# stone-d-chen/ffvvc

Measured on AMD Instinct MI355X. Metric: decoded frames/sec (4K/8K 10-bit VVC) per GPU, higher is better.
Workload: dtype u16

## Files before the change

### ffvvc_amd/csrc/intra.hip

```cpp
#include <type_traits>
#include "common.hpp"
#include "pk16.hpp"
#include "wave.hpp"
#include "runtime.hpp"
#include "resid_math.hpp"
#include "../../include/vvc_mi355.h"

namespace vvc355 {

#define VVC355_TABLE(type, name, count) __device__ static const type i_tab_##name[count] __attribute__((aligned(16)))
#include "tables.inc"
#undef VVC355_TABLE

#ifdef VVC355_RECON_PROF
__device__ unsigned long long vvc355_recon_prof[64];
__device__ __forceinline__ unsigned long long *rprof_lds() { __shared__ unsigned long long p[64]; return p; }
#define RPROF_NOW() wall_clock64()
#define RPROF_ADD(slot, t0) do { unsigned long long *p_ = rprof_lds(); p_[slot] = p_[slot] + (unsigned long long)(wall_clock64() - (t0)); } while (0)
#define RPROF_INC(slot) do { unsigned long long *p_ = rprof_lds(); p_[slot] = p_[slot] + 1ull; } while (0)
__device__ unsigned long long vvc355_recon_trace[4096 * 8];
#define RTRACE(rs, slot, v) do { vvc355_recon_trace[((rs) & 4095) * 8 + (slot)] = (unsigned long long)(v); } while (0)
#else
#define RTRACE(rs, slot, v) do { } while (0)
#define RPROF_NOW() 0ull
// ... 126 lines not shown
    int base;
    __device__ __forceinline__ int ld(int off) const { return p[base + off]; }
    __device__ __forceinline__ void st(int off, int v) const { p[base + off] = (uint16_t)v; }
    __device__ __forceinline__ LPix at(int off) const { return LPix{ p, base + off }; }
    __device__ __forceinline__ void st4(int off, int a, int b, int c, int d) const
    {
        uint32_t *q = (uint32_t *)(p + base + off);
        q[0] = (uint32_t)a | ((uint32_t)b << 16);
        q[1] = (uint32_t)c | ((uint32_t)d << 16);
    }
    __device__ __forceinline__ void ld4(int off, int *v) const
    {
        const uint32_t *q = (const uint32_t *)(p + base + off);
        const uint32_t a = q[0], b = q[1];
        v[0] = (int)(a & 0xffff); v[1] = (int)(a >> 16); v[2] = (int)(b & 0xffff); v[3] = (int)(b >> 16);
    }
};

template <int BD> __device__ __forceinline__ GPix<BD> pick3(int c, GPix<BD> a, GPix<BD> b, GPix<BD> d) { return GPix<BD>{ c == 0 ? a.p : c == 1 ? b.p : d.p }; }
__device__ __forceinline__ LPix pick3(int c, LPix a, LPix b, LPix d) { return LPix{ a.p, c == 0 ? a.base : c == 1 ? b.base : d.base }; }
__device__ __forceinline__ StripRef pick3(int c, StripRef a, StripRef b, StripRef d)
{
    return StripRef{ a.p + (c == 0 ? 0 : c == 1 ? (int)(b.p - a.p) : (int)(d.p - a.p)), c == 0 ? a.pitch : c == 1 ? b.pitch : d.pitch, c == 0 ? a.x0s : c == 1 ? b.x0s : d.x0s, false };
}

struct IntraTabsLds {
    uint32_t angle_inv[32];
    uint32_t luma_filter[64];
    uint8_t mip4[1024], mip8[1024], mip16[2688];
};
struct GTabs {
    __device__ __forceinline__ uint32_t angle_inv(int aidx) const { return intra_angle_entry(aidx); }
    __device__ __forceinline__ uint32_t filt4(int e) const { uint32_t d; __builtin_memcpy(&d, i_tab_intra_luma_filter + e * 4, 4); return d; }
    __device__ __forceinline__ const uint8_t *mip(int size_id) const
    {
        return size_id == 0 ? i_tab_mip_matrix_4x4 : size_id == 1 ? i_tab_mip_matrix_8x8 : i_tab_mip_matrix_16x16;
    }
};
struct LTabs {
    const IntraTabsLds *t;
    __device__ __forceinline__ uint32_t angle_inv(int aidx) const { return (uint32_t)__builtin_amdgcn_readfirstlane((int)t->angle_inv[aidx]); }
    __device__ __forceinline__ uint32_t filt4(int e) const { return t->luma_filter[e]; }
    __device__ __forceinline__ const uint8_t *mip(int size_id) const { return size_id == 0 ? t->mip4 : size_id == 1 ? t->mip8 : t->mip16; }
};
struct LTabsLane {
    const IntraTabsLds *t;
// ... 1243 lines not shown
}


namespace vvc355 {

struct ReconLds {
    uint16_t arr[3][4][kEdgeLen];
    int scratch[3][16];
    int prm[2][8];
    uint32_t rmap[2][2][2][32];
    uint32_t cmdbuf[2][64 * 10];
    int luma_done;
    int bc[8];
    IntraTabsLds tabs;
};
struct ReconCtx { int ctb_up, ctb_left, ctb_up_left, end_of_tiles_x, ox, oy; };

__device__ __forceinline__ int recon_run(uint32_t line, int from)
{
    const uint32_t m = (uint32_t)__builtin_amdgcn_readfirstlane((int)line) >> from;
    return m == ~0u ? 32 : __builtin_ctz(~m);
}
typedef uint32_t ReconMaps[2][2][32];
__device__ int recon_top_available(const vvc355_recon_frame &f, const ReconCtx &cx, const ReconMaps &rmap, int cu_x0, int x, int y, int target, int c_idx)
{
    const int hs = c_idx ? f.hs : 0, vs = c_idx ? f.vs : 0;
    const int end_of_ctb_x = ((cu_x0 >> f.ctb_log2) + 1) << f.ctb_log2;
    const int y0b = y & ((1 << (f.ctb_log2 - vs)) - 1);
    const int max_x = min(f.width, end_of_ctb_x) >> hs;
    if (!y0b) {
        if (!cx.ctb_up)
            return 0;
        target = min(target, (cx.end_of_tiles_x >> hs) - x);
        if (f.wpp)
            target = min(target, (end_of_ctb_x >> hs) - x);
        return target;
    }
    target = max(0, min(target, max_x - x));
    const int ux = ((x << hs) - cx.ox) >> 2, uy = (((y - 1) << vs) - cx.oy) >> 2;
    const int end = (cx.ox + ((ux + recon_run(rmap[c_idx > 0][0][uy], ux)) << 2)) >> hs;
    return max(0, min(target, end - x));
}
__device__ int recon_left_available(const vvc355_recon_frame &f, const ReconCtx &cx, const ReconMaps &rmap, int cu_y0, int x, int y, int target, int c_idx)
{
    const int hs = c_idx ? f.hs : 0, vs = c_idx ? f.vs : 0;
    const int x0b = x & ((1 << (f.ctb_log2 - hs)) - 1);
    const int end_of_ctb_y = ((cu_y0 >> f.ctb_log2) + 1) << f.ctb_log2;
    const int max_y = min(f.height, end_of_ctb_y) >> vs;
    if (!x0b && !cx.ctb_left)
        return 0;
    target = max(0, min(target, max_y - y));
    if (!x0b)
        return target;
    const int ux = (((x - 1) << hs) - cx.ox) >> 2, uy = ((y << vs) - cx.oy) >> 2;
    const int end = (cx.oy + ((uy + recon_run(rmap[c_idx > 0][1][ux], uy)) << 2)) >> vs;
    return max(0, min(target, end - y));
}
__host__ __device__ inline int wide_angle_mode(int isp_split, int c_idx, int tb_w, int tb_h, int cb_w, int cb_h, int mode)
{
    const int nw = (!isp_split || c_idx) ? tb_w : cb_w, nh = (!isp_split || c_idx) ? tb_h : cb_h;
    const int d = ilog2i(nw) - ilog2i(nh), wh_ratio = d < 0 ? -d : d;
    const int mx = wh_ratio > 1 ? 8 + 2 * wh_ratio : 8, mn = wh_ratio > 1 ? 60 - 2 * wh_ratio : 60;
    if (nw > nh && mode >= 2 && mode < mx)
        return mode + 65;
    if (nh > nw && mode <= 66 && mode > mn)
        return mode - 67;
// ... 189 lines not shown
        group_sync<64>();
    }
    asm volatile("s_waitcnt vmcnt(0)" ::: "memory");
    __syncthreads();
    if (role == 0) {
        __builtin_amdgcn_fence(__ATOMIC_RELEASE, "agent");
        asm volatile("s_waitcnt vmcnt(0)" ::: "memory");
        __hip_atomic_store(&state[kReconFlags + n_ctus + rs], 1, __ATOMIC_RELAXED, __HIP_MEMORY_SCOPE_AGENT);
        __hip_atomic_store(&state[kReconFlags + rs], 1, __ATOMIC_RELAXED, __HIP_MEMORY_SCOPE_AGENT);
        RTRACE(rs, 2, wall_clock64()); RTRACE(rs, 4, wall_clock64()); RTRACE(rs, 5, wall_clock64());
        RTRACE(rs, 6, ctu.flags | ((unsigned long long)ctu.n_cmd << 8)); 
    }
}

template <int BD, bool TILE>
__device__ __forceinline__ bool recon_one_ctu(const vvc355_recon_frame &f, ReconLds &L, uint16_t *tiles, const int role, const int tid)
{
    using px_t = typename Px<BD>::type;
    using PX = typename std::conditional<TILE, LPix, GPix<BD>>::type;
    VVC355_GLOBAL int *state = (VVC355_GLOBAL int *)f.state;
    if (role == 0) {
        const int t = __hip_atomic_fetch_add(&state[0], tid == 0 ? 1 : 0, __ATOMIC_RELAXED, __HIP_MEMORY_SCOPE_AGENT);
        L.bc[0] = __builtin_amdgcn_readfirstlane(t);
        recon_luma_done_set(L, 0);
    }
    __syncthreads();
    const int ticket = __builtin_amdgcn_readfirstlane(L.bc[0]);
    if (ticket >= f.n_work)
        return false;
    const int rs = __builtin_amdgcn_readfirstlane(gld<int>((const int *)f.order + ticket));
    const vvc355_recon_ctu *ctus = (const vvc355_recon_ctu *)f.ctus;
    const vvc355_recon_ctu ctu = load_uniform(ctus + rs);
    const int ncx = f.ctb_width, ry = rs / ncx, rx = rs - ry * ncx;
    const int ctb = 1 << f.ctb_log2;
    ReconCtx cx;
    {
        const int16_t *slice_idx = (const int16_t *)f.slice_idx, *col_bd = (const int16_t *)f.ctb_to_col_bd, *row_bd = (const int16_t *)f.ctb_to_row_bd;
        const bool left_tile = rx > 0 && gld<int16_t>(col_bd + rx) != gld<int16_t>(col_bd + rx - 1);
        const bool upper_tile = ry > 0 && gld<int16_t>(row_bd + ry) != gld<int16_t>(row_bd + ry - 1);
        const bool upper_slice = ry > 0 && gld<int16_t>(slice_idx + rs) != gld<int16_t>(slice_idx + rs - ncx);
        cx.end_of_tiles_x = f.width;
        if (gld<int16_t>(col_bd + rx) != gld<int16_t>(col_bd + rx + 1))
            cx.end_of_tiles_x = min(rx * ctb + ctb, f.width);
        cx.ctb_left = rx > 0 && !left_tile;
        cx.ctb_up = ry > 0 && !upper_tile && !upper_slice;
        cx.ctb_up_left = cx.ctb_left && cx.ctb_up;
        cx.ox = rx * ctb; cx.oy = ry * ctb;
// ... 11 lines not shown
    const int cw0 = min(ctb, f.width - rx * ctb), ch0 = min(ctb, f.height - ry * ctb);
    if constexpr (TILE) {
#pragma unroll
        for (int c = 0; c < 3; c++) {
            const int sh = c ? 1 : 0, pitch = c ? kBodyChromaP : kBodyLumaP, spitch = c ? kStripChromaP : kStripLumaP;
            const int ox = (rx * ctb) >> sh, oy = (ry * ctb) >> sh;
            if ((c == 0) == (role == 0)) {
                if (c == 0)
                    recon_body_load<BD, 5>(tiles + kTileOff[c], pitch, (const uint8_t *)f.plane[c], f.stride[c], ox, oy, cw0, ch0, f.width, f.height, tid);
                else
                    recon_body_load<BD, 4>(tiles + kTileOff[c], pitch, (const uint8_t *)f.plane[c], f.stride[c], ox, oy, cw0 >> 1, ch0 >> 1, f.width >> 1, f.height >> 1, tid);
            }
            const LPix px{ tiles, kTileOff[c] - oy * pitch + (kApr - ox) };
            const StripRef sx{ tiles + kStripOff[c], spitch, ox - kApr, false };
            if (c == 0) { pl0 = px; st0 = sx; } else if (c == 1) { pl1 = px; st1 = sx; } else { pl2 = px; st2 = sx; }
        }
        ps0 = kBodyLumaP; ps1 = kBodyChromaP;
    }
    const vvc355_recon_cmd *cmds = (const vvc355_recon_cmd *)f.cmds + ctu.first_cmd;
    const int ctb_mask = ctb - 1;
    constexpr int CMD_DW = (int)sizeof(vvc355_recon_cmd) / 4;
    static_assert(CMD_DW == 10, "cmdbuf holds windows of 10-dword commands");
    const uint32_t n_cmd = ctu.n_cmd;
    uint16_t (*arr)[kEdgeLen] = L.arr[role];
    const LTabs tabs{ &L.tabs };
    VVC355_LDS uint32_t *cbuf = (VVC355_LDS uint32_t *)L.cmdbuf[role];
    auto load_window = [&](uint32_t base, uint32_t *all_kinds, auto plan) -> unsigned long long {
        const uint32_t n_dw = min(64u, n_cmd - base) * CMD_DW;
        const uint32_t *g = (const uint32_t *)(cmds + base);
        uint32_t v[CMD_DW];
#pragma unroll
        for (int u = 0; u < CMD_DW; u++)
            v[u] = (uint32_t)tid + 64u * u < n_dw ? gld<uint32_t>(g + tid + 64 * u) : 0u;
#pragma unroll
        for (int u = 0; u < CMD_DW; u++)
            cbuf[tid + 64 * u] = v[u];
        group_sync<64>();
        const uint32_t kinds = cbuf[tid * CMD_DW + 6];
        *all_kinds = kinds;
        const unsigned long long m = __ballot(base + (uint32_t)tid < n_cmd && ((((kinds >> 16) & 0xff) > 0) == (role == 1)) && ((kinds >> 8) & 0xff) != VVC355_RECON_MARK);
        if constexpr (decltype(plan)::value) {
            const bool mine = (m >> tid) & 1;
            ReconPlan P;
            if (mine) {
                uint32_t q[CMD_DW], qn[CMD_DW] = {};
#pragma unroll
                for (int i = 0; i < CMD_DW; i++) q[i] = cbuf[tid * CMD_DW + i];
                bool twin = false;
                if (TILE && tid < 63 && ((m >> (tid + 1)) & 1)) {
#pragma unroll
                    for (int i = 2; i < 9; i++) qn[i] = cbuf[(tid + 1) * CMD_DW + i];
                    twin = recon_plan_twin(q, qn);
                }
                const ReconPlanFrame pf = { f.hs, f.vs, f.ctb_log2, { ps0, ps1 }, TILE };
                P = recon_plan(q, twin, pf, cx, LTabsLane{ &L.tabs });
            }
            group_sync<64>();
            if (mine) {
#pragma unroll
                for (int i = 0; i < CMD_DW; i++) cbuf[tid * CMD_DW + i] = P.d[i];
            }
            group_sync<64>();
        }
        return m;
    };
    {
        ReconMaps &rmap = L.rmap[role];
        ((uint32_t *)rmap)[tid] = 0;
        ((uint32_t *)rmap)[tid + 64] = 0;
        uint32_t *cmd_dw = (uint32_t *)cmds;
        for (uint32_t base = 0; base < n_cmd; base += 64) {
            uint32_t kinds;
            (void)load_window(base, &kinds, std::false_type{});
            const uint32_t kind_l = (kinds >> 8) & 0xff, type_l = ((kinds >> 16) & 0xff) > 0;
            const bool in_l = base + (uint32_t)tid < n_cmd;
            const bool mine = type_l == (uint32_t)role;
            const bool scaled_l = in_l && mine && kind_l == VVC355_RECON_RESID && ((cbuf[tid * CMD_DW + 8] >> 8) & 8);
            unsigned long long todo = __ballot(in_l && ((kind_l == VVC355_RECON_MARK && (role == 1 || type_l == 0)) ||
                                                        (mine && (kind_l == VVC355_RECON_PRED || kind_l == VVC355_RECON_CCLM)) || scaled_l));
            while (todo) {
                const int k = __builtin_ctzll(todo);
                todo &= todo - 1;
                const uint32_t q2 = __builtin_amdgcn_readfirstlane(cbuf[k * CMD_DW + 2]), q3 = __builtin_amdgcn_readfirstlane(cbuf[k * CMD_DW + 3]);
                const uint32_t q4 = __builtin_amdgcn_readfirstlane(cbuf[k * CMD_DW + 4]), q6 = __builtin_amdgcn_readfirstlane(cbuf[k * CMD_DW + 6]);
                const int x0 = (int16_t)(q2 & 0xffff), y0 = (int16_t)(q2 >> 16), cw_ = (int16_t)(q3 & 0xffff), ch_ = (int16_t)(q3 >> 16);
                const int cu_x0 = (int16_t)(q4 & 0xffff), cu_y0 = (int16_t)(q4 >> 16);
                const int kind = (q6 >> 8) & 0xff, c_idx = (q6 >> 16) & 0xff;
                if (kind == VVC355_RECON_MARK) {
                    const int ux = (x0 - cx.ox) >> 2, uy = (y0 - cx.oy) >> 2, uw = max(1, cw_ >> 2), uh = max(1, ch_ >> 2);
                    const int i = tid & 31, t = tid >> 5;
                    const int span = t ? uw : uh, first = t ? ux : uy, len = t ? uh : uw, at = t ? uy : ux;
                    if (i < span)
                        rmap[c_idx > 0][t][first + i] |= (len >= 32 ? ~0u : ((1u << len) - 1)) << at;
                    __builtin_amdgcn_fence(__ATOMIC_RELEASE, "wavefront");
                    continue;
                }
// ... 1 lines not shown
                if (kind == VVC355_RECON_PRED) {
                    const int hs = c_idx ? f.hs : 0, vs = c_idx ? f.vs : 0;
                    dw9 = (uint32_t)(uint16_t)__builtin_amdgcn_readfirstlane(recon_left_available(f, cx, rmap, cu_y0, x0 >> hs, y0 >> vs, 16384, c_idx)) |
                          (uint32_t)(uint16_t)__builtin_amdgcn_readfirstlane(recon_top_available(f, cx, rmap, cu_x0, x0 >> hs, y0 >> vs, 16384, c_idx)) << 16;
                } else if (kind == VVC355_RECON_CCLM) {
                    dw9 = (uint32_t)(uint16_t)__builtin_amdgcn_readfirstlane(recon_left_available(f, cx, rmap, cu_y0, x0 >> f.hs, y0 >> f.vs, 16384, 1)) |
                          (uint32_t)(uint16_t)__builtin_amdgcn_readfirstlane(recon_top_available(f, cx, rmap, cu_x0, x0 >> f.hs, y0 >> f.vs, 16384, 1)) << 16;
                    bits = (__builtin_amdgcn_readfirstlane(recon_left_available(f, cx, rmap, cu_y0, x0, y0, 1, 0)) != 0 ? 1u : 0u) |
                           (__builtin_amdgcn_readfirstlane(recon_top_available(f, cx, rmap, cu_x0, x0, y0, 1, 0)) != 0 ? 2u : 0u);
                } else {
                    const int size_y = min(ctb, 64), xv = cu_x0 & ~(size_y - 1), yv = cu_y0 & ~(size_y - 1);
                    bits = (__builtin_amdgcn_readfirstlane(recon_left_available(f, cx, rmap, cu_y0, xv, yv, 1, 0)) != 0 ? 1u : 0u) |
                           (__builtin_amdgcn_readfirstlane(recon_top_available(f, cx, rmap, cu_x0, xv, yv, 1, 0)) != 0 ? 2u : 0u);
                }
                if (tid == 0) {
                    uint32_t *g = cmd_dw + (size_t)(base + k) * CMD_DW;
                    gst<uint32_t>(g + 9, dw9);
                    gst<uint8_t>((uint8_t *)(g + 8) + 2, (uint8_t)bits);
                }
            }
        }
        asm volatile("s_waitcnt vmcnt(0)" ::: "memory");
    }
    const unsigned long long t_wait = RPROF_NOW();
    if (role == 0) { RTRACE(rs, 0, wall_clock64()); RTRACE(rs, 6, ctu.flags | ((unsigned long long)ctu.n_cmd << 8)); }
    {
        const int n_ctus = ncx * f.ctb_height;
        const int dep[4] = { rx > 0 ? rs - 1 : -1, (rx > 0 && ry > 0) ? rs - ncx - 1 : -1, ry > 0 ? rs - ncx : -1, (ry > 0 && rx + 1 < ncx) ? rs - ncx + 1 : -1 };
#pragma unroll
        for (int d = 0; d < 4; d++) {
            if (dep[d] < 0 || __builtin_amdgcn_readfirstlane(gld<uint32_t>(&ctus[dep[d]].n_cmd)) == 0)
                continue;
            if (role == 0 && (__builtin_amdgcn_readfirstlane(gld<uint32_t>(&ctus[dep[d]].flags)) & VVC355_RECON_CTU_LIGHT))
                continue;
            VVC355_GLOBAL int *flag = &state[kReconFlags + (role == 0 ? n_ctus : 0) + dep[d]];
            while (__builtin_amdgcn_readfirstlane(__hip_atomic_load(flag, __ATOMIC_RELAXED, __HIP_MEMORY_SCOPE_AGENT)) == 0)
                __builtin_amdgcn_s_sleep(4);
        }
        __builtin_amdgcn_fence(__ATOMIC_ACQUIRE, "agent");
        asm volatile("s_waitcnt vmcnt(0)" ::: "memory");
    }
    RPROF_ADD(1 + 32 * role, t_wait);
    RPROF_INC(0 + 32 * role);
    RTRACE(rs, role ? 3 : 1, wall_clock64());
    const unsigned long long t_load = RPROF_NOW();
    if constexpr (TILE) {
#pragma unroll
        for (int c = 0; c < 3; c++) {
            const int sh = c ? 1 : 0;
            if ((c == 0) == (role == 0))
                recon_edges_load<BD>(tiles + kTileOff[c], c ? kBodyChromaP : kBodyLumaP, tiles + kStripOff[c], c ? kStripChromaP : kStripLumaP, (const uint8_t *)f.plane[c], f.stride[c],
                                     (rx * ctb) >> sh, (ry * ctb) >> sh, ctb >> sh, ch0 >> sh, f.width >> sh, f.height >> sh, tid);
        }
        asm volatile("s_waitcnt vmcnt(0)" ::: "memory");
        group_sync<64>();
    } else {
        pl0 = GPix<BD>{ (uint8_t *)f.plane[0] }; pl1 = GPix<BD>{ (uint8_t *)f.plane[1] }; pl2 = GPix<BD>{ (uint8_t *)f.plane[2] };
        ps0 = f.stride[0] / (int)sizeof(px_t); ps1 = f.stride[1] / (int)sizeof(px_t);
    }

    RPROF_ADD(2 + 32 * role, t_load);
    const unsigned long long t_loop = RPROF_NOW();
#ifdef VVC355_RECON_PROF
    const long long c_loop = clock64();
#endif
    uint32_t win = (uint32_t)0 - 64u, kinds_unused;
    unsigned long long mask = 0;
    auto advance = [&]() -> int {
        while (!mask) {
            if (win + 64 >= n_cmd)
                return -1;
            win += 64;
            mask = load_window(win, &kinds_unused, std::true_type{});
        }
        const int bit = __builtin_ctzll(mask);
        mask &= mask - 1;
        return (int)win + bit;
    };
    auto load_cmd = [&](int idx) -> uint32_t { return cbuf[(idx - (int)win) * CMD_DW + min(tid, CMD_DW - 1)]; };
    int i0 = -1;
    auto shift = [&]() {
        i0 = advance();
        if (role == 0)
            recon_luma_done_set(L, i0 >= 0 ? i0 : (int)n_cmd);
    };
    int4 pre[4] = {};
    int pre_k = -1;
    int lmcs_xv = -1, lmcs_yv = -1, lmcs_scale = 0;
    int n_shift = 1;
    for (;;) {
        do shift(); while (--n_shift);
        if (i0 < 0)
            break;
        n_shift = 1;
        const uint32_t k = (uint32_t)i0;
        const int i1 = mask ? (int)win + __builtin_ctzll(mask) : -1;
        const uint32_t d0 = load_cmd(i0), d1 = i1 >= 0 ? load_cmd(i1) : 0u;
        uint32_t p[CMD_DW];
#pragma unroll
        for (int i = 0; i < CMD_DW; i++) p[i] = (uint32_t)__builtin_amdgcn_readlane((int)d0, i);
        const int kind = (int)((p[6] >> 8) & 0xff);
        if (i1 >= 0) {
            const uint32_t n6 = (uint32_t)__builtin_amdgcn_readlane((int)d1, 6);
            if (((n6 >> 8) & 0xff) == VVC355_RECON_RESID && pre_k != i0) {
                const uint64_t ptr = (uint32_t)__builtin_amdgcn_readlane((int)d1, 0) | ((uint64_t)(uint32_t)__builtin_amdgcn_readlane((int)d1, 1) << 32);
                const uint32_t wh = (uint32_t)__builtin_amdgcn_readlane((int)d1, 3);
                const int nn = (int)(wh & 0xffff) * (int)(wh >> 16);
#pragma unroll
                for (int u = 0; u < 4; u++)
                    if (tid * 4 + 256 * u < nn)
                        pre[u] = gld<int4>((const int *)ptr + tid * 4 + 256 * u);
                pre_k = i1;
            }
        }
        const unsigned long long t_cmd = RPROF_NOW();
        if (kind == VVC355_RECON_PRED) {
            const IntraSetup su = recon_plan_setup(p);
            const uint32_t fl = p[8] >> 16;
            RPROF_ADD(6 + 32 * role, t_cmd);
            if (TILE && (fl & kPlanTwin)) {
                if constexpr (TILE) {
                    const int half = tid >> 5;
                    const LPix plane2{ pl1.p, half ? pl2.base : pl1.base };
                    StripRef sr2{ st1.p + (half ? (int)(st2.p - st1.p) : 0), st1.pitch, st1.x0s, (fl & kPlanStrip) != 0 };
                    intra_pred_run<BD, 32>(su, plane2, ps1, L.arr[1 + half], L.scratch[1 + half], tid & 31, sr2, tabs);
                    group_sync<64>();
                    n_shift = 2;
                }
            } else {
                const PX plane = pick3(su.c_idx, pl0, pl1, pl2);
                StripRef sr = pick3(su.c_idx, st0, st1, st2);
                sr.on = (fl & kPlanStrip) != 0;
                intra_pred_run<BD, 64>(su, plane, su.c_idx ? ps1 : ps0, arr, L.scratch[role], tid, sr, tabs);
                if (TILE) group_sync<64>(); else recon_sync_mem();
            }
        } else if (kind == VVC355_RECON_CCLM) {
            while (recon_luma_done_get(L) < (int)k)
                __builtin_amdgcn_s_sleep(1);
            group_sync<64>();
            vvc355_cclm_job j = {};
            j.x0 = (int16_t)(p[2] & 0xffff); j.y0 = (int16_t)(p[2] >> 16); j.width = (int16_t)(p[3] & 0xffff); j.height = (int16_t)(p[3] >> 16);
            j.top_avail_c = (int16_t)(p[9] >> 16);
            j.left_avail_c = (int16_t)(p[9] & 0xffff);
            j.mode = (uint8_t)(p[6] & 0xff); j.hs = f.hs; j.vs = f.vs;
            j.avail_l = (uint8_t)(p[7] & 0xff);
            j.avail_t = (uint8_t)((p[7] >> 8) & 0xff);
            j.collocated = f.collocated;
            j.ctu_boundary = (uint8_t)((p[7] >> 16) & 0xff);
            StripRef s0 = st0, s1 = st1, s2 = st2;
            s0.on = s1.on = s2.on = TILE && j.ctu_boundary;
            cclm_body<BD, 64>(j, pl0, ps0, pl1, pl2, ps1, ps1, L.prm[1], tid, s0, s1, s2);
            if (TILE) group_sync<64>(); else recon_sync_mem();
        } else if (kind == VVC355_RECON_CIIP) {
            const int c_idx = (int)((p[4] >> 8) & 0xff), lw = (int)(p[4] & 0xff), w = 1 << lw, n = (int)p[5];
            const int stride = c_idx ? ps1 : ps0, iw = (int)((p[4] >> 16) & 0xff);
            const PX dst = pick3(c_idx, pl0, pl1, pl2).at((int)p[2]);
            const uint8_t *inter = (const uint8_t *)(p[0] | ((uint64_t)p[1] << 32));
            for (int i = tid; i < n; i += 64) {
                const int o = (i >> lw) * stride + (i & (w - 1));
                dst.st(o, (dst.ld(o) * iw + ld_px<BD>(inter, i) * (4 - iw) + 2) >> 2);
            }
            if (TILE) group_sync<64>(); else recon_sync_mem();
        } else {
            const int c_idx = (int)((p[4] >> 8) & 0xff), lw = (int)(p[4] & 0xff), w = 1 << lw, n = (int)p[5];
            const int stride = c_idx ? ps1 : ps0, joint = (int)((p[4] >> 16) & 0xff);
            const PX dst = pick3(c_idx, pl0, pl1, pl2).at((int)p[2]);
            const int *res = (const int *)(p[0] | ((uint64_t)p[1] << 32));
            const bool have = pre_k == (int)k;
            const bool scaled = (p[4] >> 24) != 0;
            const int xv = (int16_t)(p[7] & 0xffff), yv = (int16_t)(p[7] >> 16);
            if (scaled && (lmcs_xv != xv || lmcs_yv != yv)) {
                while (recon_luma_done_get(L) < (int)k)
                    __builtin_amdgcn_s_sleep(1);
                group_sync<64>();
                const int size_y = min(ctb, 64);
                lmcs_xv = xv; lmcs_yv = yv;
                const bool avail_t = (p[8] >> 17) & 1, avail_l = (p[8] >> 16) & 1;
                StripRef s0 = st0;
                s0.on = TILE && (lmcs_yv & ctb_mask) == 0;
                int v = 0;
                if (tid < size_y) {
                    if (avail_l)
                        v += pl0.ld((lmcs_yv + min(tid, min(f.height - lmcs_yv, size_y) - 1)) * ps0 + lmcs_xv - 1);
                    if (avail_t) {
                        const int xx = lmcs_xv + min(tid, min(f.width - lmcs_xv, size_y) - 1);
                        v += s0.on ? s0.at(xx, -1) : pl0.ld((lmcs_yv - 1) * ps0 + xx);
                    }
                }
#pragma unroll
                for (int sft = 32; sft; sft >>= 1)
                    v += __shfl_xor(v, sft, 64);
                const int cnt = (avail_l ? size_y : 0) + (avail_t ? size_y : 0);
                const int avg = cnt ? (v + (cnt >> 1)) >> ilog2i(cnt) : 1 << (BD - 1);
                lmcs_scale = lmcs_scale_of_avg((const vvc355_lmcs_model *)f.lmcs_model, avg, tid);
            }
            auto resid_of = [&](int r) {
                if (joint & 1)
                    r = (r * ((joint & 2) ? -1 : 1)) >> ((joint >> 2) & 1);
                if (scaled) {
                    const int v = clip_intp2(r, BD);
                    r = v > 0 ? (v * lmcs_scale + (1 << 10)) >> 11 : -((-v * lmcs_scale + (1 << 10)) >> 11);
                }
                return r;
            };
            auto add4 = [&](int i, const int4 r4) {
                const int r[4] = { r4.x, r4.y, r4.z, r4.w };
                const int o = (i >> lw) * stride + (i & (w - 1));
                int d[4];
                dst.ld4(o, d);
#pragma unroll
                for (int q = 0; q < 4; q++)
                    d[q] = clip_px<BD>(d[q] + resid_of(r[q]));
                dst.st4(o, d[0], d[1], d[2], d[3]);
            };
            if (w < 4) {
                for (int i = tid; i < n; i += 64) {
                    const int o = (i >> lw) * stride + (i & (w - 1));
                    dst.st(o, clip_px<BD>(dst.ld(o) + resid_of(gld<int>(res + i))));
                }
            } else {
#pragma unroll
                for (int u = 0; u < 4; u++) {
                    const int i = tid * 4 + 256 * u;
                    if (i < n)
                        add4(i, have ? pre[u] : gld<int4>(res + i));
                }
                for (int i = tid * 4 + 1024; i < n; i += 256)
                    add4(i, gld<int4>(res + i));
            }
            if (TILE) group_sync<64>(); else recon_sync_mem();
        }
        RPROF_ADD(9 + kind + 32 * role, t_cmd);
        RPROF_INC(17 + kind + 32 * role);
    }
    RPROF_ADD(3 + 32 * role, t_loop);
#ifdef VVC355_RECON_PROF
    { unsigned long long *p_ = rprof_lds(); p_[7 + 32 * role] = p_[7 + 32 * role] + (unsigned long long)(clock64() - c_loop); }
#endif
    if (role == 0) {
        if constexpr (TILE) {
            const int nk = cw0 >> 2, nr = ch0;
            recon_tile_store<BD, 5>(tiles + kTileOff[0], kBodyLumaP, (uint8_t *)f.plane[0], f.stride[0], rx * ctb, ry * ctb, max(nr - kApr, 0), nr, 0, nk, tid);
            recon_tile_store<BD, 0>(tiles + kTileOff[0], kBodyLumaP, (uint8_t *)f.plane[0], f.stride[0], rx * ctb, ry * ctb, 0, max(nr - kApr, 0), nk - 1, nk, tid);
        }
        asm volatile("s_waitcnt vmcnt(0)" ::: "memory");
        __builtin_amdgcn_fence(__ATOMIC_RELEASE, "agent");
        asm volatile("s_waitcnt vmcnt(0)" ::: "memory");
        __hip_atomic_store(&state[kReconFlags + ncx * f.ctb_height + rs], 1, __ATOMIC_RELAXED, __HIP_MEMORY_SCOPE_AGENT);
        RTRACE(rs, 2, wall_clock64());
    } else {
        RTRACE(rs, 4, wall_clock64());
    }
    const unsigned long long t_join = RPROF_NOW();
    __syncthreads();
    RPROF_ADD(4 + 32 * role, t_join);
    const unsigned long long t_store = RPROF_NOW();
    if constexpr (TILE) {
#pragma unroll
        for (int c = 0; c < 3; c++) {
            const int sh = c ? 1 : 0, pitch = c ? kBodyChromaP : kBodyLumaP, nk = cw0 >> (2 + sh), nr = ch0 >> sh;
            if ((c == 0) != (role == 0))
                continue;
            uint8_t *plane = (uint8_t *)f.plane[c];
            if (c == 0) {
            } else {
                recon_tile_store<BD, 4>(tiles + kTileOff[c], pitch, plane, f.stride[c], (rx * ctb) >> sh, (ry * ctb) >> sh, max(nr - kApr, 0), nr, 0, nk, tid);
                recon_tile_store<BD, 0>(tiles + kTileOff[c], pitch, plane, f.stride[c], (rx * ctb) >> sh, (ry * ctb) >> sh, 0, max(nr - kApr, 0), nk - 1, nk, tid);
            }
        }
    }
    asm volatile("s_waitcnt vmcnt(0)" ::: "memory");
    __syncthreads();
    if (role == 0) {
        __builtin_amdgcn_fence(__ATOMIC_RELEASE, "agent");
        asm volatile("s_waitcnt vmcnt(0)" ::: "memory");
// ... 111 lines not shown
```

Before: 612.8.

## Specialize recon command walk per role at compile time

Wraps the per-CTU wait, edge load, command loop and luma store in a generic lambda instantiated separately for the luma role and the chroma role, so role checks and plane/stride selection (pick_role) become compile-time constants. It also force-inlines the top/left availability helpers and initializes the luma-done marker to -1 instead of 0. The aim is to cut divergent branching, register pressure and scalar overhead in the hot command loop. In exchange it roughly doubles code size and may raise instruction-cache pressure. The -1 init also changes CCLM/LMCS wait semantics for the first command.

After: 630.8 (median of 6 runs). +2.9%, better.

```diff
diff --git a/ffvvc_amd/csrc/intra.hip b/ffvvc_amd/csrc/intra.hip
--- a/ffvvc_amd/csrc/intra.hip
+++ b/ffvvc_amd/csrc/intra.hip
@@ -172,6 +172,14 @@
 __device__ __forceinline__ StripRef pick3(int c, StripRef a, StripRef b, StripRef d)
 {
     return StripRef{ a.p + (c == 0 ? 0 : c == 1 ? (int)(b.p - a.p) : (int)(d.p - a.p)), c == 0 ? a.pitch : c == 1 ? b.pitch : d.pitch, c == 0 ? a.x0s : c == 1 ? b.x0s : d.x0s, false };
+}
+template <int ROLE, int BD> __device__ __forceinline__ GPix<BD> pick_role(int c, GPix<BD> a, GPix<BD> b, GPix<BD> d) { return GPix<BD>{ ROLE == 0 ? a.p : c == 1 ? b.p : d.p }; }
+template <int ROLE> __device__ __forceinline__ LPix pick_role(int c, LPix a, LPix b, LPix d) { return LPix{ a.p, ROLE == 0 ? a.base : c == 1 ? b.base : d.base }; }
+template <int ROLE> __device__ __forceinline__ StripRef pick_role(int c, StripRef a, StripRef b, StripRef d)
+{
+    if (ROLE == 0)
+        return StripRef{ a.p, a.pitch, a.x0s, false };
+    return StripRef{ b.p + (c == 1 ? 0 : (int)(d.p - b.p)), c == 1 ? b.pitch : d.pitch, c == 1 ? b.x0s : d.x0s, false };
 }
 
 struct IntraTabsLds {
@@ -1461,7 +1469,7 @@
     return m == ~0u ? 32 : __builtin_ctz(~m);
 }
 typedef uint32_t ReconMaps[2][2][32];
-__device__ int recon_top_available(const vvc355_recon_frame &f, const ReconCtx &cx, const ReconMaps &rmap, int cu_x0, int x, int y, int target, int c_idx)
+__device__ __forceinline__ int recon_top_available(const vvc355_recon_frame &f, const ReconCtx &cx, const ReconMaps &rmap, int cu_x0, int x, int y, int target, int c_idx)
 {
     const int hs = c_idx ? f.hs : 0, vs = c_idx ? f.vs : 0;
     const int end_of_ctb_x = ((cu_x0 >> f.ctb_log2) + 1) << f.ctb_log2;
@@ -1480,7 +1488,7 @@
     const int end = (cx.ox + ((ux + recon_run(rmap[c_idx > 0][0][uy], ux)) << 2)) >> hs;
     return max(0, min(target, end - x));
 }
-__device__ int recon_left_available(const vvc355_recon_frame &f, const ReconCtx &cx, const ReconMaps &rmap, int cu_y0, int x, int y, int target, int c_idx)
+__device__ __forceinline__ int recon_left_available(const vvc355_recon_frame &f, const ReconCtx &cx, const ReconMaps &rmap, int cu_y0, int x, int y, int target, int c_idx)
 {
     const int hs = c_idx ? f.hs : 0, vs = c_idx ? f.vs : 0;
     const int x0b = x & ((1 << (f.ctb_log2 - hs)) - 1);
@@ -1716,7 +1724,7 @@
     if (role == 0) {
         const int t = __hip_atomic_fetch_add(&state[0], tid == 0 ? 1 : 0, __ATOMIC_RELAXED, __HIP_MEMORY_SCOPE_AGENT);
         L.bc[0] = __builtin_amdgcn_readfirstlane(t);
-        recon_luma_done_set(L, 0);
+        recon_luma_done_set(L, -1);
     }
     __syncthreads();
     const int ticket = __builtin_amdgcn_readfirstlane(L.bc[0]);
@@ -1774,10 +1782,9 @@
     constexpr int CMD_DW = (int)sizeof(vvc355_recon_cmd) / 4;
     static_assert(CMD_DW == 10, "cmdbuf holds windows of 10-dword commands");
     const uint32_t n_cmd = ctu.n_cmd;
-    uint16_t (*arr)[kEdgeLen] = L.arr[role];
     const LTabs tabs{ &L.tabs };
-    VVC355_LDS uint32_t *cbuf = (VVC355_LDS uint32_t *)L.cmdbuf[role];
-    auto load_window = [&](uint32_t base, uint32_t *all_kinds, auto plan) -> unsigned long long {
+    auto load_window = [&](const int r, uint32_t base, uint32_t *all_kinds, auto plan) -> unsigned long long {
+        VVC355_LDS uint32_t *cbuf = (VVC355_LDS uint32_t *)L.cmdbuf[r];
         const uint32_t n_dw = min(64u, n_cmd - base) * CMD_DW;
         const uint32_t *g = (const uint32_t *)(cmds + base);
         uint32_t v[CMD_DW];
@@ -1790,7 +1797,7 @@
         group_sync<64>();
         const uint32_t kinds = cbuf[tid * CMD_DW + 6];
         *all_kinds = kinds;
-        const unsigned long long m = __ballot(base + (uint32_t)tid < n_cmd && ((((kinds >> 16) & 0xff) > 0) == (role == 1)) && ((kinds >> 8) & 0xff) != VVC355_RECON_MARK);
+        const unsigned long long m = __ballot(base + (uint32_t)tid < n_cmd && ((((kinds >> 16) & 0xff) > 0) == (r == 1)) && ((kinds >> 8) & 0xff) != VVC355_RECON_MARK);
         if constexpr (decltype(plan)::value) {
             const bool mine = (m >> tid) & 1;
             ReconPlan P;
@@ -1818,12 +1825,13 @@
     };
     {
         ReconMaps &rmap = L.rmap[role];
+        VVC355_LDS uint32_t *cbuf = (VVC355_LDS uint32_t *)L.cmdbuf[role];
         ((uint32_t *)rmap)[tid] = 0;
         ((uint32_t *)rmap)[tid + 64] = 0;
         uint32_t *cmd_dw = (uint32_t *)cmds;
         for (uint32_t base = 0; base < n_cmd; base += 64) {
             uint32_t kinds;
-            (void)load_window(base, &kinds, std::false_type{});
+            (void)load_window(role, base, &kinds, std::false_type{});
             const uint32_t kind_l = (kinds >> 8) & 0xff, type_l = ((kinds >> 16) & 0xff) > 0;
             const bool in_l = base + (uint32_t)tid < n_cmd;
             const bool mine = type_l == (uint32_t)role;
@@ -1871,235 +1879,249 @@
         }
         asm volatile("s_waitcnt vmcnt(0)" ::: "memory");
     }
-    const unsigned long long t_wait = RPROF_NOW();
-    if (role == 0) { RTRACE(rs, 0, wall_clock64()); RTRACE(rs, 6, ctu.flags | ((unsigned long long)ctu.n_cmd << 8)); }
-    {
-        const int n_ctus = ncx * f.ctb_height;
-        const int dep[4] = { rx > 0 ? rs - 1 : -1, (rx > 0 && ry > 0) ? rs - ncx - 1 : -1, ry > 0 ? rs - ncx : -1, (ry > 0 && rx + 1 < ncx) ? rs - ncx + 1 : -1 };
-#pragma unroll
-        for (int d = 0; d < 4; d++) {
-            if (dep[d] < 0 || __builtin_amdgcn_readfirstlane(gld<uint32_t>(&ctus[dep[d]].n_cmd)) == 0)
-                continue;
-            if (role == 0 && (__builtin_amdgcn_readfirstlane(gld<uint32_t>(&ctus[dep[d]].flags)) & VVC355_RECON_CTU_LIGHT))
-                continue;
-            VVC355_GLOBAL int *flag = &state[kReconFlags + (role == 0 ? n_ctus : 0) + dep[d]];
-            while (__builtin_amdgcn_readfirstlane(__hip_atomic_load(flag, __ATOMIC_RELAXED, __HIP_MEMORY_SCOPE_AGENT)) == 0)
-                __builtin_amdgcn_s_sleep(4);
-        }
-        __builtin_amdgcn_fence(__ATOMIC_ACQUIRE, "agent");
-        asm volatile("s_waitcnt vmcnt(0)" ::: "memory");
-    }
-    RPROF_ADD(1 + 32 * role, t_wait);
-    RPROF_INC(0 + 32 * role);
-    RTRACE(rs, role ? 3 : 1, wall_clock64());
-    const unsigned long long t_load = RPROF_NOW();
-    if constexpr (TILE) {
-#pragma unroll
-        for (int c = 0; c < 3; c++) {
-            const int sh = c ? 1 : 0;
-            if ((c == 0) == (role == 0))
-                recon_edges_load<BD>(tiles + kTileOff[c], c ? kBodyChromaP : kBodyLumaP, tiles + kStripOff[c], c ? kStripChromaP : kStripLumaP, (const uint8_t *)f.plane[c], f.stride[c],
-                                     (rx * ctb) >> sh, (ry * ctb) >> sh, ctb >> sh, ch0 >> sh, f.width >> sh, f.height >> sh, tid);
-        }
-        asm volatile("s_waitcnt vmcnt(0)" ::: "memory");
-        group_sync<64>();
-    } else {
-        pl0 = GPix<BD>{ (uint8_t *)f.plane[0] }; pl1 = GPix<BD>{ (uint8_t *)f.plane[1] }; pl2 = GPix<BD>{ (uint8_t *)f.plane[2] };
-        ps0 = f.stride[0] / (int)sizeof(px_t); ps1 = f.stride[1] / (int)sizeof(px_t);
-    }
-
-    RPROF_ADD(2 + 32 * role, t_load);
-    const unsigned long long t_loop = RPROF_NOW();
+    auto walk = [&](auto role_c) __attribute__((always_inline)) {
+        constexpr int kRole = decltype(role_c)::value;
+        uint16_t (*arr)[kEdgeLen] = L.arr[kRole];
+        VVC355_LDS uint32_t *cbuf = (VVC355_LDS uint32_t *)L.cmdbuf[kRole];
+        const unsigned long long t_wait = RPROF_NOW();
+        if (kRole == 0) { RTRACE(rs, 0, wall_clock64()); RTRACE(rs, 6, ctu.flags | ((unsigned long long)ctu.n_cmd << 8)); }
+        {
+            const int n_ctus = ncx * f.ctb_height;
+            const int dep[4] = { rx > 0 ? rs - 1 : -1, (rx > 0 && ry > 0) ? rs - ncx - 1 : -1, ry > 0 ? rs - ncx : -1, (ry > 0 && rx + 1 < ncx) ? rs - ncx + 1 : -1 };
+#pragma unroll
+            for (int d = 0; d < 4; d++) {
+                if (dep[d] < 0 || __builtin_amdgcn_readfirstlane(gld<uint32_t>(&ctus[dep[d]].n_cmd)) == 0)
+                    continue;
+                if (kRole == 0 && (__builtin_amdgcn_readfirstlane(gld<uint32_t>(&ctus[dep[d]].flags)) & VVC355_RECON_CTU_LIGHT))
+                    continue;
+                VVC355_GLOBAL int *flag = &state[kReconFlags + (kRole == 0 ? n_ctus : 0) + dep[d]];
+                while (__builtin_amdgcn_readfirstlane(__hip_atomic_load(flag, __ATOMIC_RELAXED, __HIP_MEMORY_SCOPE_AGENT)) == 0)
+                    __builtin_amdgcn_s_sleep(4);
+            }
+            __builtin_amdgcn_fence(__ATOMIC_ACQUIRE, "agent");
+            asm volatile("s_waitcnt vmcnt(0)" ::: "memory");
+        }
+        RPROF_ADD(1 + 32 * kRole, t_wait);
+        RPROF_INC(0 + 32 * kRole);
+        RTRACE(rs, kRole ? 3 : 1, wall_clock64());
+        const unsigned long long t_load = RPROF_NOW();
+        if constexpr (TILE) {
+#pragma unroll
+            for (int c = 0; c < 3; c++) {
+                const int sh = c ? 1 : 0;
+                if ((c == 0) == (kRole == 0))
+                    recon_edges_load<BD>(tiles + kTileOff[c], c ? kBodyChromaP : kBodyLumaP, tiles + kStripOff[c], c ? kStripChromaP : kStripLumaP, (const uint8_t *)f.plane[c], f.stride[c],
+                                         (rx * ctb) >> sh, (ry * ctb) >> sh, ctb >> sh, ch0 >> sh, f.width >> sh, f.height >> sh, tid);
+            }
+            asm volatile("s_waitcnt vmcnt(0)" ::: "memory");
+            group_sync<64>();
+        } else {
+            pl0 = GPix<BD>{ (uint8_t *)f.plane[0] }; pl1 = GPix<BD>{ (uint8_t *)f.plane[1] }; pl2 = GPix<BD>{ (uint8_t *)f.plane[2] };
+            ps0 = f.stride[0] / (int)sizeof(px_t); ps1 = f.stride[1] / (int)sizeof(px_t);
+        }
+
+        RPROF_ADD(2 + 32 * kRole, t_load);
+        const unsigned long long t_loop = RPROF_NOW();
 #ifdef VVC355_RECON_PROF
-    const long long c_loop = clock64();
+        const long long c_loop = clock64();
 #endif
-    uint32_t win = (uint32_t)0 - 64u, kinds_unused;
-    unsigned long long mask = 0;
-    auto advance = [&]() -> int {
-        while (!mask) {
-            if (win + 64 >= n_cmd)
-                return -1;
-            win += 64;
-            mask = load_window(win, &kinds_unused, std::true_type{});
-        }
-        const int bit = __builtin_ctzll(mask);
-        mask &= mask - 1;
-        return (int)win + bit;
-    };
-    auto load_cmd = [&](int idx) -> uint32_t { return cbuf[(idx - (int)win) * CMD_DW + min(tid, CMD_DW - 1)]; };
-    int i0 = -1;
-    auto shift = [&]() {
-        i0 = advance();
-        if (role == 0)
-            recon_luma_done_set(L, i0 >= 0 ? i0 : (int)n_cmd);
-    };
-    int4 pre[4] = {};
-    int pre_k = -1;
-    int lmcs_xv = -1, lmcs_yv = -1, lmcs_scale = 0;
-    int n_shift = 1;
-    for (;;) {
-        do shift(); while (--n_shift);
-        if (i0 < 0)
-            break;
-        n_shift = 1;
-        const uint32_t k = (uint32_t)i0;
-        const int i1 = mask ? (int)win + __builtin_ctzll(mask) : -1;
-        const uint32_t d0 = load_cmd(i0), d1 = i1 >= 0 ? load_cmd(i1) : 0u;
-        uint32_t p[CMD_DW];
-#pragma unroll
-        for (int i = 0; i < CMD_DW; i++) p[i] = (uint32_t)__builtin_amdgcn_readlane((int)d0, i);
-        const int kind = (int)((p[6] >> 8) & 0xff);
-        if (i1 >= 0) {
-            const uint32_t n6 = (uint32_t)__builtin_amdgcn_readlane((int)d1, 6);
-            if (((n6 >> 8) & 0xff) == VVC355_RECON_RESID && pre_k != i0) {
-                const uint64_t ptr = (uint32_t)__builtin_amdgcn_readlane((int)d1, 0) | ((uint64_t)(uint32_t)__builtin_amdgcn_readlane((int)d1, 1) << 32);
-                const uint32_t wh = (uint32_t)__builtin_amdgcn_readlane((int)d1, 3);
-                const int nn = (int)(wh & 0xffff) * (int)(wh >> 16);
-#pragma unroll
-                for (int u = 0; u < 4; u++)
-                    if (tid * 4 + 256 * u < nn)
-                        pre[u] = gld<int4>((const int *)ptr + tid * 4 + 256 * u);
-                pre_k = i1;
-            }
-        }
-        const unsigned long long t_cmd = RPROF_NOW();
-        if (kind == VVC355_RECON_PRED) {
-            const IntraSetup su = recon_plan_setup(p);
-            const uint32_t fl = p[8] >> 16;
-            RPROF_ADD(6 + 32 * role, t_cmd);
-            if (TILE && (fl & kPlanTwin)) {
-                if constexpr (TILE) {
-                    const int half = tid >> 5;
-                    const LPix plane2{ pl1.p, half ? pl2.base : pl1.base };
-                    StripRef sr2{ st1.p + (half ? (int)(st2.p - st1.p) : 0), st1.pitch, st1.x0s, (fl & kPlanStrip) != 0 };
-                    intra_pred_run<BD, 32>(su, plane2, ps1, L.arr[1 + half], L.scratch[1 + half], tid & 31, sr2, tabs);
-                    group_sync<64>();
-                    n_shift = 2;
+        uint32_t win = (uint32_t)0 - 64u, kinds_unused;
+        unsigned long long mask = 0;
+        auto advance = [&]() -> int {
+            while (!mask) {
+                if (win + 64 >= n_cmd)
+                    return -1;
+                win += 64;
+                const unsigned long long t_win = RPROF_NOW();
+                mask = load_window(kRole, win, &kinds_unused, std::true_type{});
+                RPROF_ADD(8 + 32 * kRole, t_win);
+                RPROF_INC(16 + 32 * kRole);
+            }
+            const int bit = __builtin_ctzll(mask);
+            mask &= mask - 1;
+            return (int)win + bit;
+        };
+        auto load_cmd = [&](int idx) -> uint32_t { return cbuf[(idx - (int)win) * CMD_DW + min(tid, CMD_DW - 1)]; };
+        int i0 = -1;
+        auto shift = [&]() {
+            i0 = advance();
+            if (kRole == 0)
+                recon_luma_done_set(L, i0 >= 0 ? i0 : (int)n_cmd);
+        };
+        int4 pre[4] = {};
+        int pre_k = -1;
+        int lmcs_xv = -1, lmcs_yv = -1, lmcs_scale = 0;
+        int n_shift = 1;
+        for (;;) {
+            do shift(); while (--n_shift);
+            if (i0 < 0)
+                break;
+            n_shift = 1;
+            const uint32_t k = (uint32_t)i0;
+            const int i1 = mask ? (int)win + __builtin_ctzll(mask) : -1;
+            const uint32_t d0 = load_cmd(i0), d1 = i1 >= 0 ? load_cmd(i1) : 0u;
+            uint32_t p[CMD_DW];
+#pragma unroll
+            for (int i = 0; i < CMD_DW; i++) p[i] = (uint32_t)__builtin_amdgcn_readlane((int)d0, i);
+            const int kind = (int)((p[6] >> 8) & 0xff);
+            if (i1 >= 0) {
+                const uint32_t n6 = (uint32_t)__builtin_amdgcn_readlane((int)d1, 6);
+                if (((n6 >> 8) & 0xff) == VVC355_RECON_RESID && pre_k != i0) {
+                    const uint64_t ptr = (uint32_t)__builtin_amdgcn_readlane((int)d1, 0) | ((uint64_t)(uint32_t)__builtin_amdgcn_readlane((int)d1, 1) << 32);
+                    const uint32_t wh = (uint32_t)__builtin_amdgcn_readlane((int)d1, 3);
+                    const int nn = (int)(wh & 0xffff) * (int)(wh >> 16);
+#pragma unroll
+                    for (int u = 0; u < 4; u++)
+                        if (tid * 4 + 256 * u < nn)
+                            pre[u] = gld<int4>((const int *)ptr + tid * 4 + 256 * u);
+                    pre_k = i1;
                 }
-            } else {
-                const PX plane = pick3(su.c_idx, pl0, pl1, pl2);
-                StripRef sr = pick3(su.c_idx, st0, st1, st2);
-                sr.on = (fl & kPlanStrip) != 0;
-                intra_pred_run<BD, 64>(su, plane, su.c_idx ? ps1 : ps0, arr, L.scratch[role], tid, sr, tabs);
-                if (TILE) group_sync<64>(); else recon_sync_mem();
-            }
-        } else if (kind == VVC355_RECON_CCLM) {
-            while (recon_luma_done_get(L) < (int)k)
-                __builtin_amdgcn_s_sleep(1);
-            group_sync<64>();
-            vvc355_cclm_job j = {};
-            j.x0 = (int16_t)(p[2] & 0xffff); j.y0 = (int16_t)(p[2] >> 16); j.width = (int16_t)(p[3] & 0xffff); j.height = (int16_t)(p[3] >> 16);
-            j.top_avail_c = (int16_t)(p[9] >> 16);
-            j.left_avail_c = (int16_t)(p[9] & 0xffff);
-            j.mode = (uint8_t)(p[6] & 0xff); j.hs = f.hs; j.vs = f.vs;
-            j.avail_l = (uint8_t)(p[7] & 0xff);
-            j.avail_t = (uint8_t)((p[7] >> 8) & 0xff);
-            j.collocated = f.collocated;
-            j.ctu_boundary = (uint8_t)((p[7] >> 16) & 0xff);
-            StripRef s0 = st0, s1 = st1, s2 = st2;
-            s0.on = s1.on = s2.on = TILE && j.ctu_boundary;
-            cclm_body<BD, 64>(j, pl0, ps0, pl1, pl2, ps1, ps1, L.prm[1], tid, s0, s1, s2);
-            if (TILE) group_sync<64>(); else recon_sync_mem();
-        } else if (kind == VVC355_RECON_CIIP) {
-            const int c_idx = (int)((p[4] >> 8) & 0xff), lw = (int)(p[4] & 0xff), w = 1 << lw, n = (int)p[5];
-            const int stride = c_idx ? ps1 : ps0, iw = (int)((p[4] >> 16) & 0xff);
-            const PX dst = pick3(c_idx, pl0, pl1, pl2).at((int)p[2]);
-            const uint8_t *inter = (const uint8_t *)(p[0] | ((uint64_t)p[1] << 32));
-            for (int i = tid; i < n; i += 64) {
-                const int o = (i >> lw) * stride + (i & (w - 1));
-                dst.st(o, (dst.ld(o) * iw + ld_px<BD>(inter, i) * (4 - iw) + 2) >> 2);
-            }
-            if (TILE) group_sync<64>(); else recon_sync_mem();
-        } else {
-            const int c_idx = (int)((p[4] >> 8) & 0xff), lw = (int)(p[4] & 0xff), w = 1 << lw, n = (int)p[5];
-            const int stride = c_idx ? ps1 : ps0, joint = (int)((p[4] >> 16) & 0xff);
-            const PX dst = pick3(c_idx, pl0, pl1, pl2).at((int)p[2]);
-            const int *res = (const int *)(p[0] | ((uint64_t)p[1] << 32));
-            const bool have = pre_k == (int)k;
-            const bool scaled = (p[4] >> 24) != 0;
-            const int xv = (int16_t)(p[7] & 0xffff), yv = (int16_t)(p[7] >> 16);
-            if (scaled && (lmcs_xv != xv || lmcs_yv != yv)) {
+            }
+            const unsigned long long t_cmd = RPROF_NOW();
+            if (kind == VVC355_RECON_PRED) {
+                IntraSetup su = recon_plan_setup(p);
+                if (kRole == 0)
+                    su.c_idx = 0;
+                const uint32_t fl = p[8] >> 16;
+                RPROF_ADD(6 + 32 * kRole, t_cmd);
+                if (kRole == 1 && TILE && (fl & kPlanTwin)) {
+                    if constexpr (TILE) {
+                        const int half = tid >> 5;
+                        const LPix plane2{ pl1.p, half ? pl2.base : pl1.base };
+                        StripRef sr2{ st1.p + (half ? (int)(st2.p - st1.p) : 0), st1.pitch, st1.x0s, (fl & kPlanStrip) != 0 };
+                        intra_pred_run<BD, 32>(su, plane2, ps1, L.arr[1 + half], L.scratch[1 + half], tid & 31, sr2, tabs);
+                        group_sync<64>();
+                        n_shift = 2;
+                    }
+                } else {
+                    const PX plane = pick_role<kRole>(su.c_idx, pl0, pl1, pl2);
+                    StripRef sr = pick_role<kRole>(su.c_idx, st0, st1, st2);
+                    sr.on = (fl & kPlanStrip) != 0;
+                    intra_pred_run<BD, 64>(su, plane, kRole ? ps1 : ps0, arr, L.scratch[kRole], tid, sr, tabs);
+                    if (TILE) group_sync<64>(); else recon_sync_mem();
+                }
+            } else if (kRole == 1 && kind == VVC355_RECON_CCLM) {
                 while (recon_luma_done_get(L) < (int)k)
                     __builtin_amdgcn_s_sleep(1);
                 group_sync<64>();
-                const int size_y = min(ctb, 64);
-                lmcs_xv = xv; lmcs_yv = yv;
-                const bool avail_t = (p[8] >> 17) & 1, avail_l = (p[8] >> 16) & 1;
-                StripRef s0 = st0;
-                s0.on = TILE && (lmcs_yv & ctb_mask) == 0;
-                int v = 0;
-                if (tid < size_y) {
-                    if (avail_l)
-                        v += pl0.ld((lmcs_yv + min(tid, min(f.height - lmcs_yv, size_y) - 1)) * ps0 + lmcs_xv - 1);
-                    if (avail_t) {
-                        const int xx = lmcs_xv + min(tid, min(f.width - lmcs_xv, size_y) - 1);
-                        v += s0.on ? s0.at(xx, -1) : pl0.ld((lmcs_yv - 1) * ps0 + xx);
-                    }
-                }
-#pragma unroll
-                for (int sft = 32; sft; sft >>= 1)
-                    v += __shfl_xor(v, sft, 64);
-                const int cnt = (avail_l ? size_y : 0) + (avail_t ? size_y : 0);
-                const int avg = cnt ? (v + (cnt >> 1)) >> ilog2i(cnt) : 1 << (BD - 1);
-                lmcs_scale = lmcs_scale_of_avg((const vvc355_lmcs_model *)f.lmcs_model, avg, tid);
-            }
-            auto resid_of = [&](int r) {
-                if (joint & 1)
-                    r = (r * ((joint & 2) ? -1 : 1)) >> ((joint >> 2) & 1);
-                if (scaled) {
-                    const int v = clip_intp2(r, BD);
-                    r = v > 0 ? (v * lmcs_scale + (1 << 10)) >> 11 : -((-v * lmcs_scale + (1 << 10)) >> 11);
-                }
-                return r;
-            };
-            auto add4 = [&](int i, const int4 r4) {
-                const int r[4] = { r4.x, r4.y, r4.z, r4.w };
-                const int o = (i >> lw) * stride + (i & (w - 1));
-                int d[4];
-                dst.ld4(o, d);
-#pragma unroll
-                for (int q = 0; q < 4; q++)
-                    d[q] = clip_px<BD>(d[q] + resid_of(r[q]));
-                dst.st4(o, d[0], d[1], d[2], d[3]);
-            };
-            if (w < 4) {
+                vvc355_cclm_job j = {};
+                j.x0 = (int16_t)(p[2] & 0xffff); j.y0 = (int16_t)(p[2] >> 16); j.width = (int16_t)(p[3] & 0xffff); j.height = (int16_t)(p[3] >> 16);
+                j.top_avail_c = (int16_t)(p[9] >> 16);
+                j.left_avail_c = (int16_t)(p[9] & 0xffff);
+                j.mode = (uint8_t)(p[6] & 0xff); j.hs = f.hs; j.vs = f.vs;
+                j.avail_l = (uint8_t)(p[7] & 0xff);
+                j.avail_t = (uint8_t)((p[7] >> 8) & 0xff);
+                j.collocated = f.collocated;
+                j.ctu_boundary = (uint8_t)((p[7] >> 16) & 0xff);
+                StripRef s0 = st0, s1 = st1, s2 = st2;
+                s0.on = s1.on = s2.on = TILE && j.ctu_boundary;
+                cclm_body<BD, 64>(j, pl0, ps0, pl1, pl2, ps1, ps1, L.prm[1], tid, s0, s1, s2);
+                if (TILE) group_sync<64>(); else recon_sync_mem();
+            } else if (kind == VVC355_RECON_CIIP) {
+                const int c_idx = (int)((p[4] >> 8) & 0xff), lw = (int)(p[4] & 0xff), w = 1 << lw, n = (int)p[5];
+                const int stride = kRole ? ps1 : ps0, iw = (int)((p[4] >> 16) & 0xff);
+                const PX dst = pick_role<kRole>(c_idx, pl0, pl1, pl2).at((int)p[2]);
+                const uint8_t *inter = (const uint8_t *)(p[0] | ((uint64_t)p[1] << 32));
                 for (int i = tid; i < n; i += 64) {
                     const int o = (i >> lw) * stride + (i & (w - 1));
-                    dst.st(o, clip_px<BD>(dst.ld(o) + resid_of(gld<int>(res + i))));
+                    dst.st(o, (dst.ld(o) * iw + ld_px<BD>(inter, i) * (4 - iw) + 2) >> 2);
                 }
+                if (TILE) group_sync<64>(); else recon_sync_mem();
             } else {
-#pragma unroll
-                for (int u = 0; u < 4; u++) {
-                    const int i = tid * 4 + 256 * u;
-                    if (i < n)
-                        add4(i, have ? pre[u] : gld<int4>(res + i));
+                const int c_idx = (int)((p[4] >> 8) & 0xff), lw = (int)(p[4] & 0xff), w = 1 << lw, n = (int)p[5];
+                const int stride = kRole ? ps1 : ps0, joint = kRole ? (int)((p[4] >> 16) & 0xff) : 0;
+                const PX dst = pick_role<kRole>(c_idx, pl0, pl1, pl2).at((int)p[2]);
+                const int *res = (const int *)(p[0] | ((uint64_t)p[1] << 32));
+                const bool have = pre_k == (int)k;
+                const bool scaled = kRole == 1 && (p[4] >> 24) != 0;
+                const int xv = (int16_t)(p[7] & 0xffff), yv = (int16_t)(p[7] >> 16);
+                if (scaled && (lmcs_xv != xv || lmcs_yv != yv)) {
+                    while (recon_luma_done_get(L) < (int)k)
+                        __builtin_amdgcn_s_sleep(1);
+                    group_sync<64>();
+                    const int size_y = min(ctb, 64);
+                    lmcs_xv = xv; lmcs_yv = yv;
+                    const bool avail_t = (p[8] >> 17) & 1, avail_l = (p[8] >> 16) & 1;
+                    StripRef s0 = st0;
+                    s0.on = TILE && (lmcs_yv & ctb_mask) == 0;
+                    int v = 0;
+                    if (tid < size_y) {
+                        if (avail_l)
+                            v += pl0.ld((lmcs_yv + min(tid, min(f.height - lmcs_yv, size_y) - 1)) * ps0 + lmcs_xv - 1);
+                        if (avail_t) {
+                            const int xx = lmcs_xv + min(tid, min(f.width - lmcs_xv, size_y) - 1);
+                            v += s0.on ? s0.at(xx, -1) : pl0.ld((lmcs_yv - 1) * ps0 + xx);
+                        }
+                    }
+#pragma unroll
+                    for (int sft = 32; sft; sft >>= 1)
+                        v += __shfl_xor(v, sft, 64);
+                    const int cnt = (avail_l ? size_y : 0) + (avail_t ? size_y : 0);
+                    const int avg = cnt ? (v + (cnt >> 1)) >> ilog2i(cnt) : 1 << (BD - 1);
+                    lmcs_scale = lmcs_scale_of_avg((const vvc355_lmcs_model *)f.lmcs_model, avg, tid);
                 }
-                for (int i = tid * 4 + 1024; i < n; i += 256)
-                    add4(i, gld<int4>(res + i));
-            }
-            if (TILE) group_sync<64>(); else recon_sync_mem();
-        }
-        RPROF_ADD(9 + kind + 32 * role, t_cmd);
-        RPROF_INC(17 + kind + 32 * role);
-    }
-    RPROF_ADD(3 + 32 * role, t_loop);
+                auto resid_of = [&](int r) {
+                    if (joint & 1)
+                        r = (r * ((joint & 2) ? -1 : 1)) >> ((joint >> 2) & 1);
+                    if (scaled) {
+                        const int v = clip_intp2(r, BD);
+                        r = v > 0 ? (v * lmcs_scale + (1 << 10)) >> 11 : -((-v * lmcs_scale + (1 << 10)) >> 11);
+                    }
+                    return r;
+                };
+                auto add4 = [&](int i, const int4 r4) {
+                    const int r[4] = { r4.x, r4.y, r4.z, r4.w };
+                    const int o = (i >> lw) * stride + (i & (w - 1));
+                    int d[4];
+                    dst.ld4(o, d);
+#pragma unroll
+                    for (int q = 0; q < 4; q++)
+                        d[q] = clip_px<BD>(d[q] + resid_of(r[q]));
+                    dst.st4(o, d[0], d[1], d[2], d[3]);
+                };
+                if (w < 4) {
+                    for (int i = tid; i < n; i += 64) {
+                        const int o = (i >> lw) * stride + (i & (w - 1));
+                        dst.st(o, clip_px<BD>(dst.ld(o) + resid_of(gld<int>(res + i))));
+                    }
+                } else {
+#pragma unroll
+                    for (int u = 0; u < 4; u++) {
+                        const int i = tid * 4 + 256 * u;
+                        if (i < n)
+                            add4(i, have ? pre[u] : gld<int4>(res + i));
+                    }
+                    for (int i = tid * 4 + 1024; i < n; i += 256)
+                        add4(i, gld<int4>(res + i));
+                }
+                if (TILE) group_sync<64>(); else recon_sync_mem();
+            }
+            RPROF_ADD(9 + kind + 32 * kRole, t_cmd);
+            RPROF_INC(17 + kind + 32 * kRole);
+        }
+        RPROF_ADD(3 + 32 * kRole, t_loop);
 #ifdef VVC355_RECON_PROF
-    { unsigned long long *p_ = rprof_lds(); p_[7 + 32 * role] = p_[7 + 32 * role] + (unsigned long long)(clock64() - c_loop); }
+        { unsigned long long *p_ = rprof_lds(); p_[7 + 32 * kRole] = p_[7 + 32 * kRole] + (unsigned long long)(clock64() - c_loop); }
 #endif
-    if (role == 0) {
-        if constexpr (TILE) {
-            const int nk = cw0 >> 2, nr = ch0;
-            recon_tile_store<BD, 5>(tiles + kTileOff[0], kBodyLumaP, (uint8_t *)f.plane[0], f.stride[0], rx * ctb, ry * ctb, max(nr - kApr, 0), nr, 0, nk, tid);
-            recon_tile_store<BD, 0>(tiles + kTileOff[0], kBodyLumaP, (uint8_t *)f.plane[0], f.stride[0], rx * ctb, ry * ctb, 0, max(nr - kApr, 0), nk - 1, nk, tid);
-        }
-        asm volatile("s_waitcnt vmcnt(0)" ::: "memory");
-        __builtin_amdgcn_fence(__ATOMIC_RELEASE, "agent");
-        asm volatile("s_waitcnt vmcnt(0)" ::: "memory");
-        __hip_atomic_store(&state[kReconFlags + ncx * f.ctb_height + rs], 1, __ATOMIC_RELAXED, __HIP_MEMORY_SCOPE_AGENT);
-        RTRACE(rs, 2, wall_clock64());
-    } else {
-        RTRACE(rs, 4, wall_clock64());
-    }
+        if (kRole == 0) {
+            if constexpr (TILE) {
+                const int nk = cw0 >> 2, nr = ch0;
+                recon_tile_store<BD, 5>(tiles + kTileOff[0], kBodyLumaP, (uint8_t *)f.plane[0], f.stride[0], rx * ctb, ry * ctb, max(nr - kApr, 0), nr, 0, nk, tid);
+                recon_tile_store<BD, 0>(tiles + kTileOff[0], kBodyLumaP, (uint8_t *)f.plane[0], f.stride[0], rx * ctb, ry * ctb, 0, max(nr - kApr, 0), nk - 1, nk, tid);
+            }
+            asm volatile("s_waitcnt vmcnt(0)" ::: "memory");
+            __builtin_amdgcn_fence(__ATOMIC_RELEASE, "agent");
+            asm volatile("s_waitcnt vmcnt(0)" ::: "memory");
+            __hip_atomic_store(&state[kReconFlags + ncx * f.ctb_height + rs], 1, __ATOMIC_RELAXED, __HIP_MEMORY_SCOPE_AGENT);
+            RTRACE(rs, 2, wall_clock64());
+        } else {
+            RTRACE(rs, 4, wall_clock64());
+        }
+    };
+    if (role == 0)
+        walk(std::integral_constant<int, 0>{});
+    else
+        walk(std::integral_constant<int, 1>{});
     const unsigned long long t_join = RPROF_NOW();
     __syncthreads();
     RPROF_ADD(4 + 32 * role, t_join);
```
